# tjhladish/PLS

Measured on AMD Instinct MI355X. Metric: NIPALS components/sec, higher is better.
Workload: dtype f64; 1 GPU; C3: synthetic tall n=1048576 x p=512, m=1, A=20, f64, resident in HBM; algo=nipals, fuse=1, deflation_written_back_every=1, rows_per_gpu=1048576, parallelism=single GPU

## Files before the change

pls_amd/csrc/ctx.hpp:

```cpp
#pragma once

namespace {

struct DevBuf {
    void *p = nullptr;
    size_t bytes = 0;
};

struct Launch {
    int fam;
    i64 bytes;
    hipEvent_t e0, e1;
};

}

struct pls_hip_context {
    int device = 0;
    hipStream_t stream = nullptr;
    pls_hip_allreduce_fn reducer = nullptr;
    void *reducer_user = nullptr;
    int rank = 0, nranks = 1;
    double *user_red = nullptr;
    i64 user_red_count = 0;
// ... 17 lines not shown
    int num_cu = 256;
    plsh::Stager stager;
    int copy_threads = 0;
    hipStream_t copy_stream = nullptr;
    const double *pre_xx = nullptr, *pre_xy = nullptr;
    bool defer_free = false;
    std::vector<void *> graveyard;
    struct XchgIpc *xchg = nullptr;
    struct XchgEndpoint {
        bool on = false;
        int n = 0, rank = 0;
        double *const *inbox = nullptr;
        unsigned long long *const *flags = nullptr;
        unsigned long long *seq = nullptr;
        int *status = nullptr, *host_status = nullptr;
        const long long *limit = nullptr;
    } xep;
    DevBuf tailcnt;
    DevBuf resident;
    DevBuf rgflags;
    unsigned rg_epoch = 0;
    unsigned long long resident_launches = 0;
    struct Env {
        bool batch_refit = false;
        i64 batch_round = 0;
        bool tiny = true, cv_refit = false, tail = true, replica_guard = true, resident = true;
        int tail_update = 1;
        int xb4 = 1;
        int resident_gram = 1;
    } env;
    int *diverged = nullptr, *diverged_dev = nullptr;
    DevBuf guard;
};

namespace {

#define HIPCHK(ctx, call)                                                                  \
    do {                                                                                   \
        hipError_t e__ = (call);                                                           \
        if (e__ != hipSuccess) {                                                           \
            (ctx)->err = std::string(#call) + ": " + hipGetErrorString(e__);               \
            return PLS_HIP_ERR_DEVICE;                                                     \
        }                                                                                  \
    } while (0)

#define CHK(expr)                      \
// ... 109 lines not shown
```

pls_amd/csrc/fused_kernels.hpp:

```cpp
#pragma once
#include "common.hpp"
#include "exchange_kernels.hpp"
#include "update_m1.hpp"

namespace plsk {

#ifdef PLS_HIP_TESTING
__device__ unsigned long long *g_pass_stamps = nullptr;
#define PLS_STAMP(slot)                                                                                 \
    do {                                                                                                \
        if (g_pass_stamps && threadIdx.x == 0) {                                                        \
            g_pass_stamps[(size_t)blockIdx.x * 8 + (slot)] = wall_clock64();                            \
            if ((slot) == 0) {         \
                g_pass_stamps[(size_t)blockIdx.x * 8 + 4] = __builtin_amdgcn_s_getreg((31 << 11) | 20);  \
                g_pass_stamps[(size_t)blockIdx.x * 8 + 5] = __builtin_amdgcn_s_getreg((31 << 11) | 4);   \
            }                                                                                           \
        }                                                                                               \
    } while (0)
#else
#define PLS_STAMP(slot) do { } while (0)
#endif

typedef unsigned int u32x4 __attribute__((ext_vector_type(4)));

// ... 34 lines not shown
    Pack<T, V> o;
    __builtin_memcpy(&o, p, sizeof(o));
    return o;
}
template <typename T, int V>
__device__ __forceinline__ void st_pack_u(T *p, const Pack<T, V> &x) {
    __builtin_memcpy(p, &x, sizeof(x));
}

template <typename T>
__device__ __forceinline__ __amdgpu_buffer_rsrc_t score_rsrc(const T *col, i64 nvalid) {
    return __builtin_amdgcn_make_buffer_rsrc(const_cast<T *>(col), (short)0, (int)(nvalid * (i64)sizeof(T)), BUF_WORD3);
}

struct TailUpdate {
    double *XY = nullptr;
    double *W = nullptr, *P = nullptr, *Q = nullptr, *R = nullptr, *vnext = nullptr;
    int A = 0, a = 0, nipals = 0;
};

struct WalkWeights {
    int nfull = -1;
    unsigned mask = 0;
};

struct SliceTail {
    unsigned *cnt = nullptr;
    double *red = nullptr;
    int nrows = 0;
    int npush = 0;
    unsigned long long seq = 0;
    XchgPeers peers;
    TailUpdate upd;
    XchgGather gx;
};

constexpr int TAIL_MIN_WG = 32;
constexpr int TAIL_AUX_SYS = 17;

__device__ __noinline__ void tail_update_m1(const double *src, i64 stride, int n, int sys, int ok, double *XY, double *W, double *P,
                                            double *Q, double *R, double *vnext, int K, int A, int a, int nipals, double *scratch,
                                            double *wl) {
    typedef unsigned int u32x2 __attribute__((ext_vector_type(2)));
    static_assert(XCHG_MAX == 2 * RED_SLICES, "two batches of RED_SLICES loads");
    const int L = K + 1;
    update_m1<512, 1>(
        [&](int j) -> double {
// ... 140 lines not shown
            while (__hip_atomic_load(gx.flags + tid, __ATOMIC_RELAXED, __HIP_MEMORY_SCOPE_SYSTEM) < gx.seq) {
                if (wall_clock64() - t0 > gx.limit) {
                    *role = 0;
                    break;
                }
                __builtin_amdgcn_s_sleep(4);
            }
            __builtin_amdgcn_fence(__ATOMIC_ACQUIRE, "");
            asm volatile("s_waitcnt vmcnt(0)" ::: "memory");
        }
        __syncthreads();
        const int ok = *role;
        if (!ok && tid == 0) {
            *gx.status = 1;
            __hip_atomic_store(gx.host_status, 1, __ATOMIC_RELAXED, __HIP_MEMORY_SCOPE_SYSTEM);
        }
        tail_update_m1(gx.inbox, gx.cap, gx.n, 1, ok, u.XY, u.W, u.P, u.Q, u.R, u.vnext, K, u.A, u.a, u.nipals, scratch, wl);
        return;
    }
    tail_update_m1(st.red, LP, RED_SLICES, 0, 1, u.XY, u.W, u.P, u.Q, u.R, u.vnext, K, u.A, u.a, u.nipals, scratch, wl);
}

constexpr int AUX_NT = 2;

template <bool XCD, int R>
struct TileWalk {
    __device__ __forceinline__ explicit TileWalk(i64) {}
    __device__ __forceinline__ unsigned first() const { return blockIdx.x; }
    __device__ __forceinline__ unsigned step() const { return gridDim.x; }
    __device__ __forceinline__ i64 nlim(i64 N) const { return N; }
};
template <int R>
struct TileWalk<true, R> {
    i64 first_, step_, nlim_;
    __device__ __forceinline__ explicit TileWalk(i64 N) : first_(blockIdx.x), step_(gridDim.x), nlim_(N) {
        if ((gridDim.x & 7) == 0) {
            const i64 per = ((N + R - 1) / R + 7) / 8;
            first_ = (i64)(blockIdx.x & 7) * per + (blockIdx.x >> 3);
            step_ = gridDim.x >> 3;
            nlim_ = min(N, (i64)((blockIdx.x & 7) + 1) * per * R);
        }
    }
    __device__ __forceinline__ i64 first() const { return first_; }
    __device__ __forceinline__ i64 step() const { return step_; }
    __device__ __forceinline__ i64 nlim(i64) const { return nlim_; }
};
// ... 50 lines not shown
    for (int j = 0; j < CPT; ++j) pacc[j] = 0.0;
    double ss = 0.0;
    int buf = 0;
    constexpr int CGD = EDGE ? WAVE / RP : CG;
    const int cgw = EDGE ? __builtin_amdgcn_readfirstlane(cg) : 0;
    const uint32_t xoff = (uint32_t)(((i64)rp * V + (i64)(cg - cgw) * ldx) * (i64)sizeof(T));
    uint32_t doff = (DEFL && STORE) ? (uint32_t)(((i64)rp * V + (i64)cg * ldd) * (i64)sizeof(T)) : 0u;
    i64 dtile = tsd;
    if constexpr (RDST && DEFL) {
        doff = (uint32_t)(((i64)((rp * V) / rdst) * tsd + (rp * V) % rdst + (i64)cg * ldd) * (i64)sizeof(T));
        dtile = (R / rdst) * tsd;
    }
    constexpr uint32_t OOR = 0x80000000u;
    constexpr bool TBUF = DEFL && sizeof(T) == 8 && R == 32 && CPT == 16;
    const __amdgpu_buffer_rsrc_t rs_tin = score_rsrc<T>(DEFL ? tprev : tout, NV);

    TileWalk<EDGE == 2, R> walk(N);
    const int pace = rdst & 0xffff;
    constexpr bool WEIGHTED = DEFL && EDGE != 2;
    const int wfast = (WEIGHTED && wk.nfull >= 0) ? ((wk.mask >> (blockIdx.x & 7)) & 1) : 0;
    const i64 wswitch = (WEIGHTED && wk.nfull >= 0) ? (i64)wk.nfull * gridDim.x : (i64)1 << 62;
    i64 wstep = walk.step();
    bool wshared = true;
    for (i64 tile = walk.first(); tile * R < walk.nlim(N); buf ^= 1) {
        const i64 i0 = tile * R + (i64)rp * V;
        const bool rowok = (i0 < N);
        const uint32_t xo = rowok ? xoff : OOR, dof = rowok ? doff : OOR;
        int cgz = cg;
        asm volatile("" : "+v"(cgz));
        if constexpr (TILED && DEFL && STORE) {
            if (!LATE_FILL || !first_tile)
                for (int q = 0; q < pace; ++q) __builtin_amdgcn_s_sleep(1);
        }
        Pack<T, V> x[CPT];
        constexpr int GSTEP = CG * R * (int)sizeof(T);
        const int trec = K * R * (int)sizeof(T);
        if constexpr (TILED) {
            const __amdgpu_buffer_rsrc_t rs =
                __builtin_amdgcn_make_buffer_rsrc(const_cast<T *>(X + tile * tsx), (short)0, trec, BUF_WORD3);
#pragma unroll
            for (int j = 0; j < CPT; ++j) x[j] = buf_ld_so<T, V, LDAUX>(rs, xo, j * GSTEP);
            __builtin_amdgcn_sched_barrier(0);
            if constexpr (LATE_OK) {
                if (LATE_FILL && first_tile) {
                    first_tile = false;
                    if (tid < CG * CPT) {
                        vs[tid] = v_late;
                        ps[tid] = p_late;
                    }
                    __syncthreads();
                }
            }
        } else {
#pragma unroll
            for (int j = 0; j < CPT; ++j) {
                const int cols = min(CGD, K - CG * j - cgw);
                const uint32_t nrec = cols > 0 ? (uint32_t)((i64)cols * ldx * (i64)sizeof(T)) : 0u;
                const __amdgpu_buffer_rsrc_t rs = __builtin_amdgcn_make_buffer_rsrc(
                    const_cast<T *>(X + tile * tsx + (i64)(j * CG + cgw) * ldx), (short)0, (int)nrec, BUF_WORD3);
                x[j] = buf_ld<T, V, LDAUX>(rs, xo);
                __builtin_amdgcn_sched_barrier(0);
            }
        }
        if (DEFL) {
            double tp[V];
            {
                Pack<T, V> tpk;
                if constexpr (TBUF) {
                    tpk = buf_ld<T, V>(rs_tin, rowok ? (uint32_t)(i0 * (i64)sizeof(T)) : OOR);
                } else if (rowok && i0 + V <= NV) {
                    tpk = ld_pack_u<T, V>(tprev + i0);
                } else {
#pragma unroll
                    for (int e = 0; e < V; ++e) tpk.v[e] = (rowok && i0 + e < NV) ? tprev[i0 + e] : (T)0;
                }
#pragma unroll
                for (int e = 0; e < V; ++e) tp[e] = -(double)tpk.v[e];
            }
#pragma unroll
            for (int j = 0; j < CPT; ++j) {
                const double pk = ps[cgz + CG * j];
#pragma unroll
                for (int e = 0; e < V; ++e) x[j].v[e] = (T)fma(tp[e], pk, (double)x[j].v[e]);
                if constexpr (!STORE) {
                    continue;
                } else if constexpr (TILED) {
                    const __amdgpu_buffer_rsrc_t rd =
                        __builtin_amdgcn_make_buffer_rsrc(dst + tile * tsd, (short)0, trec, BUF_WORD3);
                    buf_st_so<T, V, STAUX>(rd, dof, j * GSTEP, x[j]);
                } else if constexpr (RDST) {
                    const __amdgpu_buffer_rsrc_t rd = __builtin_amdgcn_make_buffer_rsrc(
                        dst + tile * dtile + (i64)j * CG * ldd, (short)0, 0x7fffffff, BUF_WORD3);
                    buf_st<T, V, STAUX>(rd, (cg + CG * j < K) ? dof : OOR, x[j]);
                } else {
                    const int cols = min(CG, K - CG * j);
                    const uint32_t nrec = cols > 0 ? (uint32_t)((i64)cols * ldd * (i64)sizeof(T)) : 0u;
                    const __amdgpu_buffer_rsrc_t rd = __builtin_amdgcn_make_buffer_rsrc(
                        dst + tile * tsd + (i64)j * CG * ldd, (short)0, (int)nrec, BUF_WORD3);
                    buf_st<T, V, STAUX>(rd, dof, x[j]);
                }
            }
        }
        if constexpr (DEFL && STORE) __builtin_amdgcn_sched_barrier(0);
        double tp2[V];
#pragma unroll
        for (int e = 0; e < V; ++e) tp2[e] = 0.0;
#pragma unroll
        for (int j = 0; j < CPT; ++j) {
            const double vk = vs[cgz + CG * j];
#pragma unroll
            for (int e = 0; e < V; ++e) tp2[e] = fma((double)x[j].v[e], vk, tp2[e]);
        }
#pragma unroll
        for (int e = 0; e < V; ++e)
            tp2[e] = xor_range_sum<RP, WAVE>(tp2[e]);
        if (lane < RP)
#pragma unroll
            for (int e = 0; e < V; ++e) tred[buf][wv][rp * V + e] = tp2[e];
        __syncthreads();
        double t[V];
#pragma unroll
        for (int e = 0; e < V; ++e) {
            double s = 0.0;
#pragma unroll
            for (int w = 0; w < NW; ++w) s += tred[buf][w][rp * V + e];
            t[e] = (double)(T)s;
        }
        if (cg == 0 && rowok) {
            Pack<T, V> o;
#pragma unroll
            for (int e = 0; e < V; ++e) o.v[e] = (T)t[e];
            if (i0 + V <= NV) {
                st_pack_u<T, V>(tout + i0, o);
            } else {
#pragma unroll
                for (int e = 0; e < V; ++e)
                    if (i0 + e < NV) tout[i0 + e] = o.v[e];
            }
#pragma unroll
            for (int e = 0; e < V; ++e) ss = fma(t[e], t[e], ss);
        }
        if (sizeof(T) < sizeof(double)) {
#pragma unroll
            for (int j = 0; j < CPT; ++j)
#pragma unroll
                for (int e = 0; e < V; ++e) asm volatile("" : "+v"(x[j].v[e]));
        }
#pragma unroll
        for (int j = 0; j < CPT; ++j)
#pragma unroll
            for (int e = 0; e < V; ++e) pacc[j] = fma((double)x[j].v[e], t[e], pacc[j]);
        if constexpr (!WEIGHTED) {
            tile += walk.step();
            continue;
        }
        tile += wstep;
        if (wshared && tile >= wswitch) {
            if (!wfast) break;
            wshared = false;
            const int nfc = __builtin_popcount(wk.mask), below = __builtin_popcount(wk.mask & ((1u << (blockIdx.x & 7)) - 1u));
            tile = wswitch + (i64)(blockIdx.x >> 3) * nfc + below;
            wstep = (i64)(gridDim.x >> 3) * nfc;
        }
    }

    PLS_STAMP(1);
#pragma unroll
    for (int j = 0; j < CPT; ++j) {
        const double s = xor_range_sum<1, RP>(pacc[j]);
        const int k = cg + CG * j;
        if (rp == 0 && k < K) st_agent(part + (i64)blockIdx.x * K + k, s);
    }
    ss = block_sum<NW>(ss, sred);
    if (tid == 0) st_agent(sspart + blockIdx.x, ss);
    constexpr bool ONE_PER_CU = !(CPT <= 16 && !DEFL) || ONEWG;
    if (ONE_PER_CU && st.cnt) {
        asm volatile("s_waitcnt vmcnt(0)" ::: "memory");
        __syncthreads();
        static_assert(NT == 512, "tail_update_m1 plays the update's 1024 virtual threads with 512");
        PLS_STAMP(2);
        slice_tail<NT>(st, part, sspart, K, reinterpret_cast<int *>(sred + NW - 1), sred, &tred[0][0][0], vs);
    }
    PLS_STAMP(3);
}
// ... 575 lines not shown
constexpr int tile_rows() { return (512 / CGX) * (16 / (int)sizeof(T)); }

inline int tall_groups(int K) {
    return K <= 128 ? 8 : (K <= 256 ? 16 : 32);
}

template <typename T>
int fused_pass_mode(const T *X, i64 ldx, i64 N, int K, const T *Tm, i64 ldt) {
    const int CG = tall_groups(K);
    if (K > 32 * 32 || N < 1 || !elem_aligned<T>(Tm) || (N + 16) * (i64)sizeof(T) >= (1ll << 31)) return 0;
    const int e = edge_level<T>(X, ldx, CG, CG / 8);
    return e < 0 ? 0 : (e == 0 ? 1 : 2);
}
template <typename T>
bool fused_pass_covers(const T *X, i64 ldx, i64 N, int K, const T *Tm, i64 ldt) {
    return fused_pass_mode<T>(X, ldx, N, K, Tm, ldt) != 0;
}

template <typename T, int CGX = 32>
int launch_fused_pass(hipStream_t stream, int num_cu, const T *X, i64 ldx, i64 tsx, T *dst, i64 ldd, i64 tsd,
                      i64 N, int K, const double *v, const T *tprev, const double *pprev, T *tout,
                      double *part, int max_rows, double *sspart, int *nb, int *nss, int grid_hint, int rdst = 0,
                      bool src_padded = false, const SliceTail *tail = nullptr, bool *tail_used = nullptr,
                      bool *upd_done = nullptr, bool store = true) {
    constexpr int V = 16 / sizeof(T);
    constexpr int R = tile_rows<T, CGX>(), NT = 512;
    constexpr int CG = NT / (R / V);
    static_assert(CG == CGX, "tile shape");
    const bool defl = (tprev != nullptr);
    const bool stores = defl && store;
    if (!stores) dst = nullptr;
    if (!elem_aligned<T>(tout) || (defl && !elem_aligned<T>(tprev)) || (stores && !cols_aligned<T>(dst, ldd))) return 1;
    int edge = edge_level<T>(X, ldx, CG, WAVE / (R / V));
    if (edge < 0 || (edge == 0 && tsx % V != 0) || (stores && tsd % V != 0)) return 1;
    if (K > CG * ((CGX == 64 || CGX == 128 || CGX == 256 || CGX < 32 || (CGX == 512 && defl)) ? 16 : 32) || N < 1 || max_rows < 2) return 1;
    if ((N + V) * (i64)sizeof(T) >= (1ll << 31)) return 1;
    if (stores && (i64)CG * ldd * (i64)sizeof(T) >= (1ll << 31)) return 1;
    if (rdst > 0 && (CGX != 32 || !stores || rdst < V || R % rdst != 0 ||
                     ((i64)(R / rdst) * tsd + (i64)CG * ldd) * (i64)sizeof(T) >= (1ll << 31)))
        return 1;
    if (CGX > 32 && edge != 0) return 1;
    if constexpr (CGX == 32) {
        if (rdst > 0 && K <= CG * 16) return 1;
    }
    const i64 Nf = src_padded ? (N + V - 1) / V * V : N - N % V;
    i64 grid = 0;
    if (tail_used) *tail_used = false;
// ... 22 lines not shown
        if (Nf < N) {
            TailArgs<T> a;
            a.src = X; a.lds = ldx; a.tss = tsx; a.rs = R;
            if (defl) {
                if (stores) { a.dst = dst; a.ldd = ldd; a.tsd = tsd; a.rd = rdst > 0 ? rdst : R; }
                a.tprev = tprev; a.pprev = pprev;
            }
            a.v = v; a.tout = tout; a.part = part + grid * K; a.sspart = sspart + grid;
            a.row0 = Nf; a.nrows = (int)(N - Nf); a.K = K; a.zero_rows = V - a.nrows;
            launch_tail_rows(stream, a);
        }
        const bool tiled = defl && edge == 0 && rdst == 0 && ldx == R && tsx == (i64)R * K && (!stores || (ldd == R && tsd == (i64)R * K));
        WalkWeights wk;
        {
            constexpr double rho = 1.08;
            constexpr unsigned fast_mask = 0x55u;
            const int nfc = __builtin_popcount(fast_mask);
            if (defl && per_cu == 1 && grid == (i64)num_cu && grid % 8 == 0 && edge != 2 && ntiles >= 2 * grid) {
                const double share = (double)ntiles / ((double)grid * (1.0 + (rho - 1.0) * nfc / 8.0));
                wk.nfull = (int)std::max<i64>(1, std::min<i64>((i64)(share + 0.5), ntiles / grid));
                wk.mask = fast_mask;
            }
        }
        if (CGX > 32 && defl && !tiled) return 1;
#define FUSED_LAUNCH(CPT_, DEFL_, EDGE_, TILED_, STORE_, dyn_)                                                            \
    do {                                                                                                                  \
        if constexpr (!(DEFL_) && (CPT_) <= 16 && CGX <= 64 && (EDGE_) == 0) {                                            \
            if (onewg) {                                                                                                  \
                auto kfn1 = &fused_pass_kernel<T, V, R, NT, CPT_, DEFL_, AUX_NT, AUX_NT, false, EDGE_, TILED_, true>;     \
                hipLaunchKernelGGL(kfn1, g, b, dyn_, stream, X, ldx, tsx, dst, ldd, tsd, Nf, K, v, tprev, pprev, tout, part, sspart, 0, N, st, wk); \
                break;                                                                                                    \
            }                                                                                                             \
        }                                                                                                                 \
        auto kfn = &fused_pass_kernel<T, V, R, NT, CPT_, DEFL_, AUX_NT, AUX_NT, false, EDGE_, TILED_, false, STORE_>;    \
        if ((dyn_) > 48 * 1024 && !raise_dynamic_lds(reinterpret_cast<const void *>(kfn), (int)(dyn_))) return 1;         \
        hipLaunchKernelGGL(kfn, g, b, dyn_, stream, X, ldx, tsx, dst, ldd, tsd, Nf, K, v, tprev, pprev, tout, part, sspart, (TILED_) ? ((STORE_) ? 2 * (CPT_) : 0) | 0x10000 : 0, N, st, wk); \
    } while (0)
#define FUSED_EDGE(CPT_, DEFL_, STORE_, dyn_)                                                                             \
    do {                                                                                                                  \
        if constexpr (DEFL_) {                                                                                            \
            if (tiled) { FUSED_LAUNCH(CPT_, DEFL_, 0, true, STORE_, dyn_); break; }                                       \
        }                                                                                                                 \
        if constexpr (CGX <= 32) {                                                                                        \
            if (edge == 2) { FUSED_LAUNCH(CPT_, DEFL_, 2, false, STORE_, dyn_); break; }                                  \
            if (edge == 1) { FUSED_LAUNCH(CPT_, DEFL_, 1, false, STORE_, dyn_); break; }                                  \
        }                                                                                                                 \
// ... 65 lines not shown
```

pls_amd/csrc/plan_fit.hpp:

```cpp
#pragma once

namespace {

struct ResidentTurn {
    std::mutex mu;
    hipEvent_t ev[64] = {};
    bool have[64] = {};
    hipStream_t last[64] = {};
    bool any[64] = {};
};
inline ResidentTurn &resident_turns() {
    static ResidentTurn t;
    return t;
}
inline void resident_turn(pls_hip_context *c) {
    ResidentTurn &t = resident_turns();
    std::lock_guard<std::mutex> lock(t.mu);
    const int d = c->device & 63;
    if (t.have[d] && t.any[d] && t.last[d] != c->stream) (void)hipStreamWaitEvent(c->stream, t.ev[d], 0);
}
inline void resident_done(pls_hip_context *c) {
    ResidentTurn &t = resident_turns();
    std::lock_guard<std::mutex> lock(t.mu);
    const int d = c->device & 63;
// ... 378 lines not shown
            hipLaunchKernelGGL(plsk::coefficients_kernel, dim3(nblk), dim3(plsk::WG), 0, c->stream, R, Q, K, M, A, B);
            LAUNCH_CHECK(c);
        }
        if (gram && N > 0) {
            Range r_t("T = X R");
            int nss = 0;
            CHK(launch_xb<T>(c, X, ldx, N, K, R, K, A, Tm, ldt, nullptr, &nss));
        }
        return replica_guard(c, W, P, Q, R, B, K, M, A);
    }

    const T *Xc = X;
    i64 ldc = ldx, tsc = TR;
    constexpr i64 PV = 16 / (i64)sizeof(T);
    const i64 ldw = (tiled_work || retile_fit) ? WR : (N + PV - 1) / PV * PV, tsw = (tiled_work || retile_fit) ? WR * (i64)K : TR;
    bool cur_tiled = false;
    int defer_b = 0;
    for (int a = 0; a < A; ++a) {
        Range r_comp("component", a);
        bool tail_used = false, upd_done = false;
        const bool want_push = tail.cnt && xep_ok && update_is_single(K, M, A, a);
        const bool defl_pass = nipals && a > 0;
        const bool store_x = (a + 1 < A);
        const bool want_upd = tail.cnt && (c->env.tail_update == 2 || (c->env.tail_update == 1 && !defl_pass)) && M == 1 &&
                              K <= plsk::UPD1_KMAX && update_is_single(K, M, A, a) && (!c->reducer || want_push);
        tail.npush = 0;
        tail.upd = plsk::TailUpdate();
        tail.gx = plsk::XchgGather();
        if (want_push) {
            const unsigned long long seq = *c->xep.seq + 1;
            const int par = (int)(seq & 1);
            tail.npush = c->xep.n;
            tail.seq = seq;
            for (int j = 0; j < c->xep.n; ++j) {
                tail.peers.slot[j] = c->xep.inbox[j] + ((i64)par * c->xep.n + c->xep.rank) * plsk::XCHG_CAP;
                tail.peers.flag[j] = c->xep.flags[j] + par * c->xep.n + c->xep.rank;
            }
            if (want_upd) {
                plsk::XchgGather &gx = tail.gx;
                gx.inbox = c->xep.inbox[c->xep.rank] + (i64)par * c->xep.n * plsk::XCHG_CAP;
                gx.flags = c->xep.flags[c->xep.rank] + par * c->xep.n;
                gx.n = c->xep.n; gx.cap = plsk::XCHG_CAP; gx.seq = seq;
                gx.status = c->xep.status; gx.host_status = c->xep.host_status; gx.limit = *c->xep.limit;
            }
        }
        if (want_upd) {
// ... 16 lines not shown
                                      (np + 2) * (i64)K * 8;
                    Scope s(c, PLS_HIP_FAM_FUSED, bytes);
                    rc = plsk::launch_fused_defer<T>(c->stream, c->num_cu, Xc, ldc, tsc, work, ldw, tsw, N, K, v, np, pend,
                                                     store, Tm + (i64)a * ldt, part, (int)prow, sspart, &nb, &nss);
                    if (rc != 0) s.on = false;
                }
                if (rc != 0) return fail(c, PLS_HIP_ERR_DEVICE, "deferred fused pass launch failed");
                LAUNCH_CHECK(c);
                done = true;
                if (store) { Xc = work; ldc = ldw; tsc = tsw; cur_tiled = true; defer_b = a; }
                CHK(launch_reduce(c, part, nb, K, sspart, nss, red));
            } else if (fused_fit && !retile_fit) {
                int nb = 0, nss = 0;
                const T *tprev = (nipals && a > 0) ? Tm + (i64)(a - 1) * ldt : nullptr;
                const double *pprev = (nipals && a > 0) ? P + (i64)(a - 1) * K : nullptr;
                int rc;
                {
                    const i64 bytes = ((tprev && store_x) ? 2 : 1) * (i64)N * K * sizeof(T) +
                                      (tprev ? 2 : 1) * (i64)N * sizeof(T) + (tprev ? 3 : 2) * (i64)K * 8;
                    Scope s(c, PLS_HIP_FAM_FUSED, bytes);
                    if (mid_cg && a >= 2)
                        rc = plsk::launch_fused_pass<T, 64>(c->stream, c->num_cu, work, ldw, tsw, work, ldw, tsw, N, K, v,
                                                            tprev, pprev, Tm + (i64)a * ldt, part, (int)prow, sspart,
                                                            &nb, &nss, (int)c->opt_fused_grid, 0, true, &tail, &tail_used, &upd_done, store_x);
                    else {
#define TALL_PASS(CG_) plsk::launch_fused_pass<T, CG_>(c->stream, c->num_cu, Xc, ldc, tsc, (tprev && store_x) ? work : nullptr, ldw, tsw, N, K, v, tprev, \
                                                       pprev, Tm + (i64)a * ldt, part, (int)prow, sspart, &nb, &nss,                        \
                                                       (int)c->opt_fused_grid, (mid_cg && tprev && store_x) ? (int)WR : 0, Xc == work, &tail, &tail_used, &upd_done, store_x)
                        rc = tall_cg == 8 ? TALL_PASS(8) : (tall_cg == 16 ? TALL_PASS(16) : TALL_PASS(32));
#undef TALL_PASS
                    }
                    if (rc != 0) s.on = false;
                }
                if (rc == 0) {
                    LAUNCH_CHECK(c);
                    done = true;
                    if (tprev && store_x) { Xc = work; ldc = ldw; tsc = tsw; cur_tiled = tiled_work; }
                    if (!tail_used) CHK(launch_reduce(c, part, nb, K, sspart, nss, red));
                } else {
                    return fail(c, PLS_HIP_ERR_DEVICE, "fused pass launch failed");
                }
            } else if (wide_cg && (nipals ? (a >= 2 || retiled || wide_only) : true)) {
                int nb = 0, nss = 0, rc;
                const T *tprev = (nipals && a > 0) ? Tm + (i64)(a - 1) * ldt : nullptr;
                const double *pprev = (nipals && a > 0) ? P + (i64)(a - 1) * K : nullptr;
                if ((!nipals || wide_only) && a == 0 && !retiled) {
                    Scope s(c, PLS_HIP_FAM_DEFLATE, 2 * (i64)N * K * sizeof(T));
                    if (plsk::launch_retile<T>(c->stream, c->num_cu, X, ldx, work, ldw, tsw, (int)WR, N, K) != 0) {
                        s.on = false;
                        return fail(c, PLS_HIP_ERR_DEVICE, "retile launch failed");
                    }
                    LAUNCH_CHECK(c);
                }
                {
                    const i64 bytes = ((tprev && store_x) ? 2 : 1) * (i64)N * K * sizeof(T) + (tprev ? 2 : 1) * (i64)N * sizeof(T) + 3 * (i64)K * 8;
                    Scope s(c, PLS_HIP_FAM_FUSED, bytes);
#define WIDE_PASS(CG_) plsk::launch_fused_pass<T, CG_>(c->stream, c->num_cu, work, ldw, tsw, work, ldw, tsw, N, K, v, tprev, pprev, \
                                                        Tm + (i64)a * ldt, part, (int)prow, sspart, &nb, &nss, (int)c->opt_fused_grid, 0, true, \
                                                        &tail, &tail_used, &upd_done, store_x)
                    rc = wide_cg == 8 ? WIDE_PASS(8) : (wide_cg == 16 ? WIDE_PASS(16) : (wide_cg == 32 ? WIDE_PASS(32)
                         : (wide_cg == 64 ? WIDE_PASS(64) : (wide_cg == 128 ? WIDE_PASS(128) : (wide_cg == 256 ? WIDE_PASS(256) : WIDE_PASS(512))))));
#undef WIDE_PASS
                    if (rc != 0) s.on = false;
                }
                if (rc != 0) return fail(c, PLS_HIP_ERR_DEVICE, "short-tile fused pass launch failed");
                LAUNCH_CHECK(c);
                done = true;
                if (!tail_used) CHK(launch_reduce(c, part, nb, K, sspart, nss, red));
            }
            if (!done) {
                int nss = 0, nb = 0;
                bool have_t = false;
                if (nipals && a > 0) {
                    const T *tprev = Tm + (i64)(a - 1) * ldt;
                    const double *pprev = P + (i64)(a - 1) * K;
                    if (semi_fit) {
                        const i64 bytes = 2 * (i64)N * K * sizeof(T) + 2 * (i64)N * sizeof(T) + 2 * (i64)K * 8;
                        Scope s(c, PLS_HIP_FAM_DEFLATE, bytes);
                        const int rc = plsk::launch_deflate_score<T>(c->stream, c->num_cu, Xc, ldc, tsc, work, ldw, tsw,
                                                                     (int)(tiled_work ? WR : TR), N, K, tprev, pprev, v,
                                                                     Tm + (i64)a * ldt, sspart, (int)ssmax, &nss, Xc == work);
                        if (rc != 0) {
// ... 63 lines not shown
```

pls_amd/csrc/pls_hip.hip:

```cpp
#include <dlfcn.h>
#include <unistd.h>
#include <hip/hip_runtime.h>

#include <algorithm>
#include <atomic>
#include <cstdio>
#include <cstring>
#include <memory>
#include <new>
#include <string>
#include <type_traits>
#include <vector>

#include "../../include/pls_hip.h"
#include "fused_kernels.hpp"
#include "defer_kernels.hpp"
#include "small_kernels.hpp"
#include "coop_update.hpp"
#include "wide1_update.hpp"
#include "largem_kernels.hpp"
#include "tiny_kernels.hpp"
#include "resident_kernels.hpp"
#include "resident_gram.hpp"
#include "stream_kernels.hpp"
// ... 8 lines not shown
#include "host_pipeline.hpp"
#include "exchange_kernels.hpp"

using plsk::i64;

#include "ctx.hpp"
#include "launch_products.hpp"
#include "launch_update.hpp"
#include "plan_common.hpp"
#include "plan_fit.hpp"
#include "host_entry.hpp"
#include "plan_validation.hpp"
#include "plan_xdiag.hpp"

extern "C" {

int pls_hip_abi_version(void) { return PLS_HIP_ABI_VERSION; }

#ifdef PLS_HIP_TESTING
__attribute__((visibility("default"))) int pls_hip_test_set_pass_stamps(void *buf) {
    unsigned long long *p = (unsigned long long *)buf;
    return hipMemcpyToSymbol(HIP_SYMBOL(plsk::g_pass_stamps), &p, sizeof(p)) == hipSuccess ? 0 : 1;
}
#endif

int pls_hip_create(pls_hip_handle *out, int device, void *stream) {
    if (!out) return PLS_HIP_ERR_INVALID;
    *out = nullptr;
    int ndev = 0;
    if (hipGetDeviceCount(&ndev) != hipSuccess || ndev <= 0 || device < 0 || device >= ndev) {
        (void)hipGetLastError();
        return PLS_HIP_ERR_DEVICE;
    }
    hipDeviceProp_t prop;
    if (hipGetDeviceProperties(&prop, device) != hipSuccess) return PLS_HIP_ERR_DEVICE;
    if (std::strncmp(prop.gcnArchName, "gfx950", 6) != 0) return PLS_HIP_ERR_DEVICE;
    pls_hip_context *c = new (std::nothrow) pls_hip_context();
    if (!c) return PLS_HIP_ERR_ALLOC;
    {
        auto off = [](const char *name) { const char *e = getenv(name); return e && atoi(e) == 0; };
        auto on = [](const char *name) { const char *e = getenv(name); return e && atoi(e) != 0; };
        c->env.tiny = !off("PLS_HIP_TINY");
        c->env.cv_refit = on("PLS_HIP_CV_REFIT");
        c->env.batch_refit = on("PLS_HIP_BATCH_REFIT");
        if (const char *e = getenv("PLS_HIP_BATCH_ROUND")) c->env.batch_round = atoll(e);
        c->env.tail = !off("PLS_HIP_TAIL");
        {
            const char *e = getenv("PLS_HIP_TAIL");
            c->env.tail_update = e ? (atoi(e) >= 2 ? 2 : 0) : 1;
        }
        c->env.replica_guard = !off("PLS_HIP_REPLICA_GUARD");
        c->env.resident = !off("PLS_HIP_RESIDENT");
        if (const char *e = getenv("PLS_HIP_XB4")) c->env.xb4 = atoi(e);
        if (const char *e = getenv("PLS_HIP_RESIDENT_GRAM")) c->env.resident_gram = atoi(e);
    }
    c->device = device;
    c->num_cu = prop.multiProcessorCount > 0 ? prop.multiProcessorCount : 256;
    if (hipSetDevice(device) != hipSuccess) { delete c; return PLS_HIP_ERR_DEVICE; }
    c->stream = (hipStream_t)stream;
    *out = c;
    return PLS_HIP_OK;
}

int pls_hip_destroy(pls_hip_handle h) {
    if (!h) return PLS_HIP_OK;
    (void)hipSetDevice(h->device);
    (void)hipStreamSynchronize(h->stream);
    DevBuf *bufs[] = {&h->tailcnt, &h->resident, &h->rgflags, &h->zeros, &h->part, &h->sspart, &h->xbpart, &h->wide1, &h->red, &h->red2, &h->xx, &h->xyp, &h->praw, &h->xy, &h->v, &h->cs, &h->coop, &h->lm, &h->gxx, &h->gxy, &h->tab,
                      &h->cvidx, &h->cvx, &h->cvy, &h->cvws, &h->cve, &h->cvtx, &h->cvty, &h->cvtt, &h->cvm, &h->cvkeep, &h->cvred, &h->work, &h->hX, &h->hY,
                      &h->hT, &h->hW, &h->hP, &h->hQ, &h->hR, &h->hB, &h->hIn, &h->hOut, &h->valout, &h->valpart, &h->vale, &h->valacc, &h->valkeys,
                      &h->valhist, &h->xdS, &h->xdQ, &h->xdPT, &h->xdred, &h->xdtv, &h->xdoQ, &h->xdoT, &h->xdoS, &h->xdsmall,
                      &h->bws, &h->bv, &h->bred, &h->bmsg, &h->bssy, &h->bY, &h->boR, &h->boQ, &h->bott, &h->boB, &h->bossy};
    for (DevBuf *b : bufs)
        if (b->p) (void)hipFree(b->p);
    for (void *q : h->graveyard) (void)hipFree(q);
// ... 673 lines not shown
```

Measured before the change: 743.0 components/s.

## Alternate NIPALS deflation sweep direction and use cached loads at tile edges

The fused deflation pass now walks tiles in reverse on even components, so the tail of the previous sweep, which is still resident in the last-level cache, is revisited first. A configurable edge region (default 192 MiB, rounded to whole grid rounds) at the start and end of each sweep uses the default cache policy instead of non-temporal loads and stores, so leading tiles hit cache and trailing tiles stay cached for the next component. The tile body moves into an include file that is instantiated three times with different cache-hint constants, which grows code size. A standalone probe for tuning the edge policy is also added.

```diff
diff --git a/pls_amd/csrc/ctx.hpp b/pls_amd/csrc/ctx.hpp
--- a/pls_amd/csrc/ctx.hpp
+++ b/pls_amd/csrc/ctx.hpp
@@ -63,6 +63,8 @@
     unsigned rg_epoch = 0;
     unsigned long long resident_launches = 0;
     struct Env {
+        bool turnaround = true;
+        i64 turn_edge_bytes = plsk::TURN_EDGE_BYTES;
         bool batch_refit = false;
         i64 batch_round = 0;
         bool tiny = true, cv_refit = false, tail = true, replica_guard = true, resident = true;
diff --git a/pls_amd/csrc/fused_kernels.hpp b/pls_amd/csrc/fused_kernels.hpp
--- a/pls_amd/csrc/fused_kernels.hpp
+++ b/pls_amd/csrc/fused_kernels.hpp
@@ -1,4 +1,6 @@
 #pragma once
+#include <type_traits>
+
 #include "common.hpp"
 #include "exchange_kernels.hpp"
 #include "update_m1.hpp"
@@ -80,7 +82,22 @@
 struct WalkWeights {
     int nfull = -1;
     unsigned mask = 0;
+    int rev = 0;
+    int edge = 0;
 };
+
+struct Turn {
+    bool on = false;
+    bool rev = false;
+    i64 edge_bytes = 0;
+};
+
+#ifdef PLS_HIP_TESTING
+struct TurnRecord {
+    int rev = 0, edge = 0, ntiles = 0, grid = 0;
+};
+inline TurnRecord g_test_turn;
+#endif
 
 struct SliceTail {
     unsigned *cnt = nullptr;
@@ -267,6 +284,8 @@
 }
 
 constexpr int AUX_NT = 2;
+constexpr i64 TURN_EDGE_BYTES = 192ll << 20;
+constexpr bool TURN_LEAD_ST_DEFAULT = true;
 
 template <bool XCD, int R>
 struct TileWalk {
@@ -363,144 +382,38 @@
     const i64 wswitch = (WEIGHTED && wk.nfull >= 0) ? (i64)wk.nfull * gridDim.x : (i64)1 << 62;
     i64 wstep = walk.step();
     bool wshared = true;
-    for (i64 tile = walk.first(); tile * R < walk.nlim(N); buf ^= 1) {
-        const i64 i0 = tile * R + (i64)rp * V;
-        const bool rowok = (i0 < N);
-        const uint32_t xo = rowok ? xoff : OOR, dof = rowok ? doff : OOR;
-        int cgz = cg;
-        asm volatile("" : "+v"(cgz));
-        if constexpr (TILED && DEFL && STORE) {
-            if (!LATE_FILL || !first_tile)
-                for (int q = 0; q < pace; ++q) __builtin_amdgcn_s_sleep(1);
-        }
-        Pack<T, V> x[CPT];
-        constexpr int GSTEP = CG * R * (int)sizeof(T);
-        const int trec = K * R * (int)sizeof(T);
-        if constexpr (TILED) {
-            const __amdgpu_buffer_rsrc_t rs =
-                __builtin_amdgcn_make_buffer_rsrc(const_cast<T *>(X + tile * tsx), (short)0, trec, BUF_WORD3);
-#pragma unroll
-            for (int j = 0; j < CPT; ++j) x[j] = buf_ld_so<T, V, LDAUX>(rs, xo, j * GSTEP);
-            __builtin_amdgcn_sched_barrier(0);
-            if constexpr (LATE_OK) {
-                if (LATE_FILL && first_tile) {
-                    first_tile = false;
-                    if (tid < CG * CPT) {
-                        vs[tid] = v_late;
-                        ps[tid] = p_late;
-                    }
-                    __syncthreads();
-                }
+    constexpr bool TURNS = DEFL;
+    constexpr bool EDGES = TILED && DEFL && STORE;
+    const bool rev = TURNS && wk.rev;
+    const i64 ntl = (N + R - 1) / R;
+    const i64 etrail = ntl - wk.edge;
+    for (i64 pos = walk.first(); pos * R < walk.nlim(N); buf ^= 1) {
+        const i64 tile = rev ? ntl - 1 - pos : pos;
+        if constexpr (EDGES) {
+            if (pos < wk.edge) {
+                constexpr int LA = 0, SA = TURN_LEAD_ST_DEFAULT ? 0 : STAUX;
+#include "fused_pass_tile.inc"
+            } else if (pos >= etrail) {
+                constexpr int LA = 0, SA = 0;
+#include "fused_pass_tile.inc"
+            } else {
+                constexpr int LA = LDAUX, SA = STAUX;
+#include "fused_pass_tile.inc"
             }
         } else {
-#pragma unroll
-            for (int j = 0; j < CPT; ++j) {
-                const int cols = min(CGD, K - CG * j - cgw);
-                const uint32_t nrec = cols > 0 ? (uint32_t)((i64)cols * ldx * (i64)sizeof(T)) : 0u;
-                const __amdgpu_buffer_rsrc_t rs = __builtin_amdgcn_make_buffer_rsrc(
-                    const_cast<T *>(X + tile * tsx + (i64)(j * CG + cgw) * ldx), (short)0, (int)nrec, BUF_WORD3);
-                x[j] = buf_ld<T, V, LDAUX>(rs, xo);
-                __builtin_amdgcn_sched_barrier(0);
-            }
-        }
-        if (DEFL) {
-            double tp[V];
-            {
-                Pack<T, V> tpk;
-                if constexpr (TBUF) {
-                    tpk = buf_ld<T, V>(rs_tin, rowok ? (uint32_t)(i0 * (i64)sizeof(T)) : OOR);
-                } else if (rowok && i0 + V <= NV) {
-                    tpk = ld_pack_u<T, V>(tprev + i0);
-                } else {
-#pragma unroll
-                    for (int e = 0; e < V; ++e) tpk.v[e] = (rowok && i0 + e < NV) ? tprev[i0 + e] : (T)0;
-                }
-#pragma unroll
-                for (int e = 0; e < V; ++e) tp[e] = -(double)tpk.v[e];
-            }
-#pragma unroll
-            for (int j = 0; j < CPT; ++j) {
-                const double pk = ps[cgz + CG * j];
-#pragma unroll
-                for (int e = 0; e < V; ++e) x[j].v[e] = (T)fma(tp[e], pk, (double)x[j].v[e]);
-                if constexpr (!STORE) {
-                    continue;
-                } else if constexpr (TILED) {
-                    const __amdgpu_buffer_rsrc_t rd =
-                        __builtin_amdgcn_make_buffer_rsrc(dst + tile * tsd, (short)0, trec, BUF_WORD3);
-                    buf_st_so<T, V, STAUX>(rd, dof, j * GSTEP, x[j]);
-                } else if constexpr (RDST) {
-                    const __amdgpu_buffer_rsrc_t rd = __builtin_amdgcn_make_buffer_rsrc(
-                        dst + tile * dtile + (i64)j * CG * ldd, (short)0, 0x7fffffff, BUF_WORD3);
-                    buf_st<T, V, STAUX>(rd, (cg + CG * j < K) ? dof : OOR, x[j]);
-                } else {
-                    const int cols = min(CG, K - CG * j);
-                    const uint32_t nrec = cols > 0 ? (uint32_t)((i64)cols * ldd * (i64)sizeof(T)) : 0u;
-                    const __amdgpu_buffer_rsrc_t rd = __builtin_amdgcn_make_buffer_rsrc(
-                        dst + tile * tsd + (i64)j * CG * ldd, (short)0, (int)nrec, BUF_WORD3);
-                    buf_st<T, V, STAUX>(rd, dof, x[j]);
-                }
-            }
-        }
-        if constexpr (DEFL && STORE) __builtin_amdgcn_sched_barrier(0);
-        double tp2[V];
-#pragma unroll
-        for (int e = 0; e < V; ++e) tp2[e] = 0.0;
-#pragma unroll
-        for (int j = 0; j < CPT; ++j) {
-            const double vk = vs[cgz + CG * j];
-#pragma unroll
-            for (int e = 0; e < V; ++e) tp2[e] = fma((double)x[j].v[e], vk, tp2[e]);
-        }
-#pragma unroll
-        for (int e = 0; e < V; ++e)
-            tp2[e] = xor_range_sum<RP, WAVE>(tp2[e]);
-        if (lane < RP)
-#pragma unroll
-            for (int e = 0; e < V; ++e) tred[buf][wv][rp * V + e] = tp2[e];
-        __syncthreads();
-        double t[V];
-#pragma unroll
-        for (int e = 0; e < V; ++e) {
-            double s = 0.0;
-#pragma unroll
-            for (int w = 0; w < NW; ++w) s += tred[buf][w][rp * V + e];
-            t[e] = (double)(T)s;
-        }
-        if (cg == 0 && rowok) {
-            Pack<T, V> o;
-#pragma unroll
-            for (int e = 0; e < V; ++e) o.v[e] = (T)t[e];
-            if (i0 + V <= NV) {
-                st_pack_u<T, V>(tout + i0, o);
-            } else {
-#pragma unroll
-                for (int e = 0; e < V; ++e)
-                    if (i0 + e < NV) tout[i0 + e] = o.v[e];
-            }
-#pragma unroll
-            for (int e = 0; e < V; ++e) ss = fma(t[e], t[e], ss);
-        }
-        if (sizeof(T) < sizeof(double)) {
-#pragma unroll
-            for (int j = 0; j < CPT; ++j)
-#pragma unroll
-                for (int e = 0; e < V; ++e) asm volatile("" : "+v"(x[j].v[e]));
-        }
-#pragma unroll
-        for (int j = 0; j < CPT; ++j)
-#pragma unroll
-            for (int e = 0; e < V; ++e) pacc[j] = fma((double)x[j].v[e], t[e], pacc[j]);
+            constexpr int LA = LDAUX, SA = STAUX;
+#include "fused_pass_tile.inc"
+        }
         if constexpr (!WEIGHTED) {
-            tile += walk.step();
+            pos += walk.step();
             continue;
         }
-        tile += wstep;
-        if (wshared && tile >= wswitch) {
+        pos += wstep;
+        if (wshared && pos >= wswitch) {
             if (!wfast) break;
             wshared = false;
             const int nfc = __builtin_popcount(wk.mask), below = __builtin_popcount(wk.mask & ((1u << (blockIdx.x & 7)) - 1u));
-            tile = wswitch + (i64)(blockIdx.x >> 3) * nfc + below;
+            pos = wswitch + (i64)(blockIdx.x >> 3) * nfc + below;
             wstep = (i64)(gridDim.x >> 3) * nfc;
         }
     }
@@ -1122,7 +1035,7 @@
                       i64 N, int K, const double *v, const T *tprev, const double *pprev, T *tout,
                       double *part, int max_rows, double *sspart, int *nb, int *nss, int grid_hint, int rdst = 0,
                       bool src_padded = false, const SliceTail *tail = nullptr, bool *tail_used = nullptr,
-                      bool *upd_done = nullptr, bool store = true) {
+                      bool *upd_done = nullptr, bool store = true, const Turn &turn = Turn()) {
     constexpr int V = 16 / sizeof(T);
     constexpr int R = tile_rows<T, CGX>(), NT = 512;
     constexpr int CG = NT / (R / V);
@@ -1191,6 +1104,17 @@
                 wk.mask = fast_mask;
             }
         }
+        if (turn.on && defl) {
+            wk.rev = turn.rev ? 1 : 0;
+            if (tiled) {
+                const i64 round_bytes = grid * (i64)R * K * (i64)sizeof(T);
+                const i64 epos = turn.edge_bytes / round_bytes * grid;
+                wk.edge = (int)(2 * epos >= ntiles ? ntiles : epos);
+            }
+        }
+#ifdef PLS_HIP_TESTING
+        if (stores) g_test_turn = TurnRecord{wk.rev, wk.edge, (int)ntiles, (int)grid};
+#endif
         if (CGX > 32 && defl && !tiled) return 1;
 #define FUSED_LAUNCH(CPT_, DEFL_, EDGE_, TILED_, STORE_, dyn_)                                                            \
     do {                                                                                                                  \
diff --git a/pls_amd/csrc/fused_pass_tile.inc b/pls_amd/csrc/fused_pass_tile.inc
--- /dev/null
+++ b/pls_amd/csrc/fused_pass_tile.inc
@@ -0,0 +1,127 @@
+        const i64 i0 = tile * R + (i64)rp * V;
+        const bool rowok = (i0 < N);
+        const uint32_t xo = rowok ? xoff : OOR, dof = rowok ? doff : OOR;
+        int cgz = cg;
+        asm volatile("" : "+v"(cgz));
+        if constexpr (TILED && DEFL && STORE) {
+            if (!LATE_FILL || !first_tile)
+                for (int q = 0; q < pace; ++q) __builtin_amdgcn_s_sleep(1);
+        }
+        Pack<T, V> x[CPT];
+        constexpr int GSTEP = CG * R * (int)sizeof(T);
+        const int trec = K * R * (int)sizeof(T);
+        if constexpr (TILED) {
+            const __amdgpu_buffer_rsrc_t rs =
+                __builtin_amdgcn_make_buffer_rsrc(const_cast<T *>(X + tile * tsx), (short)0, trec, BUF_WORD3);
+#pragma unroll
+            for (int j = 0; j < CPT; ++j) x[j] = buf_ld_so<T, V, LA>(rs, xo, j * GSTEP);
+            __builtin_amdgcn_sched_barrier(0);
+            if constexpr (LATE_OK) {
+                if (LATE_FILL && first_tile) {
+                    first_tile = false;
+                    if (tid < CG * CPT) {
+                        vs[tid] = v_late;
+                        ps[tid] = p_late;
+                    }
+                    __syncthreads();
+                }
+            }
+        } else {
+#pragma unroll
+            for (int j = 0; j < CPT; ++j) {
+                const int cols = min(CGD, K - CG * j - cgw);
+                const uint32_t nrec = cols > 0 ? (uint32_t)((i64)cols * ldx * (i64)sizeof(T)) : 0u;
+                const __amdgpu_buffer_rsrc_t rs = __builtin_amdgcn_make_buffer_rsrc(
+                    const_cast<T *>(X + tile * tsx + (i64)(j * CG + cgw) * ldx), (short)0, (int)nrec, BUF_WORD3);
+                x[j] = buf_ld<T, V, LA>(rs, xo);
+                __builtin_amdgcn_sched_barrier(0);
+            }
+        }
+        if (DEFL) {
+            double tp[V];
+            {
+                Pack<T, V> tpk;
+                if constexpr (TBUF) {
+                    tpk = buf_ld<T, V>(rs_tin, rowok ? (uint32_t)(i0 * (i64)sizeof(T)) : OOR);
+                } else if (rowok && i0 + V <= NV) {
+                    tpk = ld_pack_u<T, V>(tprev + i0);
+                } else {
+#pragma unroll
+                    for (int e = 0; e < V; ++e) tpk.v[e] = (rowok && i0 + e < NV) ? tprev[i0 + e] : (T)0;
+                }
+#pragma unroll
+                for (int e = 0; e < V; ++e) tp[e] = -(double)tpk.v[e];
+            }
+#pragma unroll
+            for (int j = 0; j < CPT; ++j) {
+                const double pk = ps[cgz + CG * j];
+#pragma unroll
+                for (int e = 0; e < V; ++e) x[j].v[e] = (T)fma(tp[e], pk, (double)x[j].v[e]);
+                if constexpr (!STORE) {
+                    continue;
+                } else if constexpr (TILED) {
+                    const __amdgpu_buffer_rsrc_t rd =
+                        __builtin_amdgcn_make_buffer_rsrc(dst + tile * tsd, (short)0, trec, BUF_WORD3);
+                    buf_st_so<T, V, SA>(rd, dof, j * GSTEP, x[j]);
+                } else if constexpr (RDST) {
+                    const __amdgpu_buffer_rsrc_t rd = __builtin_amdgcn_make_buffer_rsrc(
+                        dst + tile * dtile + (i64)j * CG * ldd, (short)0, 0x7fffffff, BUF_WORD3);
+                    buf_st<T, V, SA>(rd, (cg + CG * j < K) ? dof : OOR, x[j]);
+                } else {
+                    const int cols = min(CG, K - CG * j);
+                    const uint32_t nrec = cols > 0 ? (uint32_t)((i64)cols * ldd * (i64)sizeof(T)) : 0u;
+                    const __amdgpu_buffer_rsrc_t rd = __builtin_amdgcn_make_buffer_rsrc(
+                        dst + tile * tsd + (i64)j * CG * ldd, (short)0, (int)nrec, BUF_WORD3);
+                    buf_st<T, V, SA>(rd, dof, x[j]);
+                }
+            }
+        }
+        if constexpr (DEFL && STORE) __builtin_amdgcn_sched_barrier(0);
+        double tp2[V];
+#pragma unroll
+        for (int e = 0; e < V; ++e) tp2[e] = 0.0;
+#pragma unroll
+        for (int j = 0; j < CPT; ++j) {
+            const double vk = vs[cgz + CG * j];
+#pragma unroll
+            for (int e = 0; e < V; ++e) tp2[e] = fma((double)x[j].v[e], vk, tp2[e]);
+        }
+#pragma unroll
+        for (int e = 0; e < V; ++e)
+            tp2[e] = xor_range_sum<RP, WAVE>(tp2[e]);
+        if (lane < RP)
+#pragma unroll
+            for (int e = 0; e < V; ++e) tred[buf][wv][rp * V + e] = tp2[e];
+        __syncthreads();
+        double t[V];
+#pragma unroll
+        for (int e = 0; e < V; ++e) {
+            double s = 0.0;
+#pragma unroll
+            for (int w = 0; w < NW; ++w) s += tred[buf][w][rp * V + e];
+            t[e] = (double)(T)s;
+        }
+        if (cg == 0 && rowok) {
+            Pack<T, V> o;
+#pragma unroll
+            for (int e = 0; e < V; ++e) o.v[e] = (T)t[e];
+            if (i0 + V <= NV) {
+                st_pack_u<T, V>(tout + i0, o);
+            } else {
+#pragma unroll
+                for (int e = 0; e < V; ++e)
+                    if (i0 + e < NV) tout[i0 + e] = o.v[e];
+            }
+#pragma unroll
+            for (int e = 0; e < V; ++e) ss = fma(t[e], t[e], ss);
+        }
+        if (sizeof(T) < sizeof(double)) {
+#pragma unroll
+            for (int j = 0; j < CPT; ++j)
+#pragma unroll
+                for (int e = 0; e < V; ++e) asm volatile("" : "+v"(x[j].v[e]));
+        }
+#pragma unroll
+        for (int j = 0; j < CPT; ++j)
+#pragma unroll
+            for (int e = 0; e < V; ++e) pacc[j] = fma((double)x[j].v[e], t[e], pacc[j]);
diff --git a/pls_amd/csrc/plan_fit.hpp b/pls_amd/csrc/plan_fit.hpp
--- a/pls_amd/csrc/plan_fit.hpp
+++ b/pls_amd/csrc/plan_fit.hpp
@@ -424,6 +424,7 @@
         const bool want_push = tail.cnt && xep_ok && update_is_single(K, M, A, a);
         const bool defl_pass = nipals && a > 0;
         const bool store_x = (a + 1 < A);
+        const plsk::Turn turn{c->env.turnaround, c->env.turnaround && a % 2 == 0, c->env.turn_edge_bytes};
         const bool want_upd = tail.cnt && (c->env.tail_update == 2 || (c->env.tail_update == 1 && !defl_pass)) && M == 1 &&
                               K <= plsk::UPD1_KMAX && update_is_single(K, M, A, a) && (!c->reducer || want_push);
         tail.npush = 0;
@@ -486,11 +487,11 @@
                     if (mid_cg && a >= 2)
                         rc = plsk::launch_fused_pass<T, 64>(c->stream, c->num_cu, work, ldw, tsw, work, ldw, tsw, N, K, v,
                                                             tprev, pprev, Tm + (i64)a * ldt, part, (int)prow, sspart,
-                                                            &nb, &nss, (int)c->opt_fused_grid, 0, true, &tail, &tail_used, &upd_done, store_x);
+                                                            &nb, &nss, (int)c->opt_fused_grid, 0, true, &tail, &tail_used, &upd_done, store_x, turn);
                     else {
 #define TALL_PASS(CG_) plsk::launch_fused_pass<T, CG_>(c->stream, c->num_cu, Xc, ldc, tsc, (tprev && store_x) ? work : nullptr, ldw, tsw, N, K, v, tprev, \
                                                        pprev, Tm + (i64)a * ldt, part, (int)prow, sspart, &nb, &nss,                        \
-                                                       (int)c->opt_fused_grid, (mid_cg && tprev && store_x) ? (int)WR : 0, Xc == work, &tail, &tail_used, &upd_done, store_x)
+                                                       (int)c->opt_fused_grid, (mid_cg && tprev && store_x) ? (int)WR : 0, Xc == work, &tail, &tail_used, &upd_done, store_x, turn)
                         rc = tall_cg == 8 ? TALL_PASS(8) : (tall_cg == 16 ? TALL_PASS(16) : TALL_PASS(32));
 #undef TALL_PASS
                     }
@@ -521,7 +522,7 @@
                     Scope s(c, PLS_HIP_FAM_FUSED, bytes);
 #define WIDE_PASS(CG_) plsk::launch_fused_pass<T, CG_>(c->stream, c->num_cu, work, ldw, tsw, work, ldw, tsw, N, K, v, tprev, pprev, \
                                                         Tm + (i64)a * ldt, part, (int)prow, sspart, &nb, &nss, (int)c->opt_fused_grid, 0, true, \
-                                                        &tail, &tail_used, &upd_done, store_x)
+                                                        &tail, &tail_used, &upd_done, store_x, turn)
                     rc = wide_cg == 8 ? WIDE_PASS(8) : (wide_cg == 16 ? WIDE_PASS(16) : (wide_cg == 32 ? WIDE_PASS(32)
                          : (wide_cg == 64 ? WIDE_PASS(64) : (wide_cg == 128 ? WIDE_PASS(128) : (wide_cg == 256 ? WIDE_PASS(256) : WIDE_PASS(512))))));
 #undef WIDE_PASS
diff --git a/pls_amd/csrc/pls_hip.hip b/pls_amd/csrc/pls_hip.hip
--- a/pls_amd/csrc/pls_hip.hip
+++ b/pls_amd/csrc/pls_hip.hip
@@ -54,6 +54,11 @@
     unsigned long long *p = (unsigned long long *)buf;
     return hipMemcpyToSymbol(HIP_SYMBOL(plsk::g_pass_stamps), &p, sizeof(p)) == hipSuccess ? 0 : 1;
 }
+__attribute__((visibility("default"))) int pls_hip_test_last_turn(int *out) {
+    if (!out) return 1;
+    out[0] = plsk::g_test_turn.rev; out[1] = plsk::g_test_turn.edge; out[2] = plsk::g_test_turn.ntiles; out[3] = plsk::g_test_turn.grid;
+    return 0;
+}
 #endif
 
 int pls_hip_create(pls_hip_handle *out, int device, void *stream) {
@@ -83,6 +88,10 @@
         }
         c->env.replica_guard = !off("PLS_HIP_REPLICA_GUARD");
         c->env.resident = !off("PLS_HIP_RESIDENT");
+        c->env.turnaround = !off("PLS_HIP_TURNAROUND");
+#ifdef PLS_HIP_TESTING
+        if (const char *e = getenv("PLS_HIP_TEST_TURN_EDGE_BYTES")) c->env.turn_edge_bytes = atoll(e);
+#endif
         if (const char *e = getenv("PLS_HIP_XB4")) c->env.xb4 = atoi(e);
         if (const char *e = getenv("PLS_HIP_RESIDENT_GRAM")) c->env.resident_gram = atoi(e);
     }
diff --git a/pls_amd/csrc/tune/turnaround_probe.hip b/pls_amd/csrc/tune/turnaround_probe.hip
--- /dev/null
+++ b/pls_amd/csrc/tune/turnaround_probe.hip
@@ -0,0 +1,136 @@
+#include <hip/hip_runtime.h>
+#include <algorithm>
+#include <cstdio>
+#include <cstdlib>
+#include <vector>
+typedef long long i64;
+typedef unsigned int u32x4 __attribute__((ext_vector_type(4)));
+#define CK(x) do { hipError_t e = (x); if (e != hipSuccess) { printf("HIP error %s at %d\n", hipGetErrorString(e), __LINE__); exit(1);} } while (0)
+
+constexpr int BUF_WORD3 = 0x00020000;
+constexpr int NTH = 512, CPT = 16;
+constexpr int TILE_BYTES = NTH * 16 * CPT;
+constexpr int GSTEP = NTH * 16;
+constexpr int POL_NT = 3;
+
+template <bool LDNT, bool STNT, bool WRITE>
+__device__ __forceinline__ void tile_body(char *p, uint32_t off, double a, double b, double &acc) {
+    const __amdgpu_buffer_rsrc_t rs = __builtin_amdgcn_make_buffer_rsrc(p, (short)0, TILE_BYTES, BUF_WORD3);
+    u32x4 x[CPT];
+#pragma unroll
+    for (int j = 0; j < CPT; ++j) x[j] = __builtin_amdgcn_raw_buffer_load_b128(rs, off, j * GSTEP, LDNT ? 2 : 0);
+    __builtin_amdgcn_sched_barrier(0);
+#pragma unroll
+    for (int j = 0; j < CPT; ++j) {
+        double d[2];
+        __builtin_memcpy(d, &x[j], 16);
+        d[0] = fma(d[0], a, b);
+        d[1] = fma(d[1], a, b);
+        if (WRITE) {
+            __builtin_memcpy(&x[j], d, 16);
+            __builtin_amdgcn_raw_buffer_store_b128(x[j], rs, off, j * GSTEP, STNT ? 2 : 0);
+        } else {
+            acc += d[0] * d[1];
+        }
+    }
+}
+
+template <bool WRITE>
+__global__ __launch_bounds__(NTH) void sweep(char *X, i64 ntiles, int reverse, int E, int lead, int trail, double a, double b,
+                                             double *sink) {
+    const uint32_t off = threadIdx.x * 16u;
+    const i64 nrounds = (ntiles + gridDim.x - 1) / gridDim.x;
+    const bool alledge = 2 * (i64)E >= nrounds;
+    double acc = 0.0;
+    i64 round = 0;
+    for (i64 pos = blockIdx.x; pos < ntiles; pos += gridDim.x, ++round) {
+        const i64 tile = reverse ? ntiles - 1 - pos : pos;
+        char *p = X + tile * TILE_BYTES;
+        const int pol = (E == 0) ? POL_NT : (alledge || round < E) ? lead : (round >= nrounds - E ? trail : POL_NT);
+        if (pol == POL_NT) tile_body<true, true, WRITE>(p, off, a, b, acc);
+        else if (pol == 0) tile_body<false, false, WRITE>(p, off, a, b, acc);
+        else if (pol == 2) tile_body<true, false, WRITE>(p, off, a, b, acc);
+        else tile_body<false, true, WRITE>(p, off, a, b, acc);
+    }
+    if (acc == 1.2345e300) sink[0] = acc;
+}
+
+struct Case {
+    const char *name;
+    bool write, alternate;
+    int lead, trail;
+    bool all;
+};
+
+int main(int argc, char **argv) {
+    const i64 mib = argc > 1 ? atoll(argv[1]) : 4096;
+    const int pairs = argc > 2 ? atoi(argv[2]) : 8;
+    const i64 bytes = mib << 20;
+    const i64 ntiles = bytes / TILE_BYTES;
+    hipDeviceProp_t prop;
+    CK(hipGetDeviceProperties(&prop, 0));
+    const int grid = prop.multiProcessorCount;
+    const double round_mb = (double)grid * TILE_BYTES / 1e6;
+    char *X;
+    double *sink;
+    CK(hipMalloc(&X, bytes));
+    CK(hipMalloc(&sink, 8));
+    CK(hipMemset(X, 0, bytes));
+    hipEvent_t e0, e1;
+    CK(hipEventCreate(&e0));
+    CK(hipEventCreate(&e1));
+    printf("# buffer %lld MiB = %lld tiles of %d KB, grid %d (one round = %.1f MB), %d timed pairs of sweeps, median of 5\n",
+           mib, ntiles, TILE_BYTES / 1024, grid, round_mb, pairs);
+
+    auto run = [&](const Case &c, int E) {
+        auto one = [&](int s) {
+            const int rev = c.alternate ? (s & 1) : 0;
+            if (c.write) hipLaunchKernelGGL(sweep<true>, dim3(grid), dim3(NTH), 0, 0, X, ntiles, rev, E, c.lead, c.trail, 1.0, 0.0, sink);
+            else hipLaunchKernelGGL(sweep<false>, dim3(grid), dim3(NTH), 0, 0, X, ntiles, rev, E, c.lead, c.trail, 1.0, 0.0, sink);
+            CK(hipGetLastError());
+        };
+        std::vector<double> ts;
+        for (int rep = 0; rep < 5; ++rep) {
+            one(0); one(1);
+            CK(hipEventRecord(e0));
+            for (int s = 0; s < 2 * pairs; ++s) one(s);
+            CK(hipEventRecord(e1));
+            CK(hipEventSynchronize(e1));
+            float ms;
+            CK(hipEventElapsedTime(&ms, e0, e1));
+            ts.push_back(ms / (2.0 * pairs));
+        }
+        std::sort(ts.begin(), ts.end());
+        return ts[2];
+    };
+
+    const Case cases[] = {
+        {"rw  lead ld=def st=def | trail ld=nt  st=def", true, true, 0, 2, false},
+        {"rw  lead ld=def st=nt  | trail ld=nt  st=def", true, true, 1, 2, false},
+        {"rw  lead ld=def st=def | trail ld=def st=def", true, true, 0, 0, false},
+        {"rw  lead ld=nt  st=def | trail ld=nt  st=def", true, true, 2, 2, false},
+        {"ro  lead ld=def        | trail ld=def       ", false, true, 0, 0, false},
+    };
+    const int edges[] = {0, 2, 4, 6, 7};
+    for (int w = 1; w >= 0; --w) {
+        const Case asc = {"ascending, all nt", w == 1, false, POL_NT, POL_NT, false};
+        const double base = run(asc, 0);
+        const double vol = (w ? 2.0 : 1.0) * bytes;
+        printf("%s ascending, all nt (the library today):          %8.4f ms/sweep  %6.0f GB/s\n", w ? "rw" : "ro", base, vol / base / 1e6);
+        for (const Case &c : cases) {
+            if (c.write != (w == 1)) continue;
+            for (int E : edges) {
+                const double t = run(c, E);
+                printf("%s  S = %3.0f MB (E = %d): %8.4f ms/sweep  %6.0f GB/s  saving %+7.1f us  %+6.2f %%\n", c.name, E * round_mb, E, t,
+                       vol / t / 1e6, (base - t) * 1e3, 100.0 * (base - t) / base);
+            }
+        }
+        const Case dasc = {"", w == 1, false, 0, 0, true}, dalt = {"", w == 1, true, 0, 0, true};
+        const int Eall = (int)((ntiles + grid - 1) / grid);
+        const double ta = run(dasc, Eall), tb = run(dalt, Eall);
+        printf("%s default policy everywhere: ascending %8.4f ms/sweep, alternating %8.4f ms/sweep (%+.1f us)\n", w ? "rw" : "ro", ta, tb, (ta - tb) * 1e3);
+        const double base2 = run(asc, 0);
+        printf("%s ascending, all nt, again (drift check):           %8.4f ms/sweep\n", w ? "rw" : "ro", base2);
+    }
+    return 0;
+}
```

After: 755.6 components/s, median of 6. +1.7%, better.
